# INK-USC/RE-Net

Hardware: NVIDIA H100
Metric: rgcn_aggregate_edge_messages_per_sec (higher is better)
Workload: dtype f32

## Files before the change

renet_b200/csrc/common.cuh:

```cuda
#pragma once
#include <cuda_runtime.h>
#include <stdint.h>
#include <stdio.h>
#include <stdarg.h>

#include "../../include/renet_b200.h"

namespace renet {

void set_error(const char* fmt, ...);
void count_launch(int n = 1);
void note_gemm_kernel(int kernel);
int last_gemm_kernel();

#define RENET_CHECK_ARG(cond, ...)                  \
  do {                                              \
    if (!(cond)) {                                  \
      ::renet::set_error(__VA_ARGS__);              \
      return RENET_ERR_INVALID_ARG;                 \
    }                                               \
  } while (0)

#define RENET_CHECK_CUDA(expr)                                                        \
  do {                                                                                \
    cudaError_t _e = (expr);                                                          \
    if (_e != cudaSuccess) {                                                          \
      ::renet::set_error("%s failed: %s (%s:%d)", #expr, cudaGetErrorString(_e),     \
                         __FILE__, __LINE__);                                         \
      return RENET_ERR_CUDA;                                                          \
    }                                                                                 \
  } while (0)

#define RENET_CHECK_LAUNCH(name)                                                      \
  do {                                                                                \
    cudaError_t _e = cudaGetLastError();                                              \
    if (_e != cudaSuccess) {                                                          \
      ::renet::set_error("launch of %s failed: %s", name, cudaGetErrorString(_e));    \
      return RENET_ERR_CUDA;                                                          \
    }                                                                                 \
    ::renet::count_launch();                                                          \
  } while (0)

constexpr int kNumSMs = 132;

__device__ __forceinline__ float4 ldg_f4(const float* p) {
  return __ldg(reinterpret_cast<const float4*>(p));
}
__device__ __forceinline__ float4 ldg_f4_stream(const float* p) {
  float4 r;
  asm volatile("ld.global.nc.L1::no_allocate.v4.f32 {%0,%1,%2,%3}, [%4];"
               : "=f"(r.x), "=f"(r.y), "=f"(r.z), "=f"(r.w)
               : "l"(p));
  return r;
}
__device__ __forceinline__ void st_f4(float* p, float4 v) { *reinterpret_cast<float4*>(p) = v; }

__device__ __forceinline__ void red_add_f4(float* p, float4 v) {
  asm volatile("red.global.add.v4.f32 [%0], {%1,%2,%3,%4};" ::"l"(p), "f"(v.x), "f"(v.y), "f"(v.z),
               "f"(v.w)
               : "memory");
}

bool deterministic();
int set_deterministic(int on);
int det_scratch(int64_t bytes, cudaStream_t stream, void** out);
int launch_sum_partials(const float* parts, int n_parts, int64_t stride, int64_t rows, int cols, float* out, int64_t ldo,
                        bool accumulate, cudaStream_t stream);
int scatter_add_rows_det(const float* src, int64_t ld, const int32_t* index, const int32_t* outer, float* dst, int64_t n_rows,
                         int d, cudaStream_t stream);

int sgemm_nn(const float* A, const int32_t* a_index, int64_t lda, const float* B, int64_t ldb, float* C,
             int64_t ldc, const float* bias, int64_t M, int32_t N, int32_t K, bool accumulate,
             cudaStream_t stream);
bool sgemm_nn_tiled_ok(const float* A, int64_t lda, const float* B, int64_t ldb, const float* C, int64_t ldc,
                       const float* bias, int32_t N, int32_t K);
int sgemm_nn_ffma(const float* A, const int32_t* a_index, int64_t lda, const float* B, int64_t ldb, float* C,
                  int64_t ldc, const float* bias, int64_t M, int32_t N, int32_t K, bool accumulate, bool naive,
                  cudaStream_t stream);
bool sgemm_tn_tiled_ok(const float* A, int64_t lda, const float* B, int64_t ldb, const float* C, int64_t ldc, int32_t M,
                       int32_t N);
int sgemm_tn(const float* A, const int32_t* a_index, int64_t lda, const float* B, int64_t ldb, float* C,
             int64_t ldc, int32_t M, int32_t N, int64_t K, bool accumulate, cudaStream_t stream, bool naive = false);
int sgemm_nt(const float* A, int64_t lda, const float* B, int64_t ldb, float* C, int64_t ldc,
             int64_t M, int32_t N, int32_t K, bool accumulate, cudaStream_t stream);

int gather_kernel_choice();
constexpr int64_t kStreamMinEdges = 16384;
constexpr int64_t kStreamMinNodes = 16384;
constexpr int64_t kStreamMaxNodes = 40960;
bool gather_use_stream(int64_t E, int64_t N);
void set_stream_debug_buffer(long long* p);

int gemm_mode();
constexpr int64_t kDedupMinRows = 16384;
int64_t umma_packed_bytes(int N, int K);
void set_gemm_debug_buffer(long long* p);
void set_weight_generation(int64_t g);
void* packed_cache_lookup(const void* const* keys, int nkeys, int64_t bytes, bool* hit);
bool umma_shape_ok(int N, int K);
int umma_pack_b(const float* B, int64_t sk, int64_t sn, int N, int K, void* Bp, int tile_offset, cudaStream_t stream);
struct EpiArgs {
  const int32_t* target;
  const float* lse;
  float* pmax;
  float* psum;
  float* tlogit;
  float* dT;
  int64_t ldT;
  float scale;
  const float* dscale;
};
int umma_gemm_prepacked_ex(const float* A, const int32_t* a_index, int64_t lda, const void* Bp, float* C, int64_t ldc,
                           const float* bias, int64_t M, int N, int K, bool accumulate, int batch, int64_t batch_a,
                           int64_t batch_bp, int64_t batch_c, int epi_mode, const EpiArgs& epi, int k_splits, int64_t split_c,
                           cudaStream_t stream);
int umma_gemm_prepacked(const float* A, const int32_t* a_index, int64_t lda, const void* Bp, float* C, int64_t ldc,
                        const float* bias, int64_t M, int N, int K, bool accumulate, int batch, int64_t batch_a,
                        int64_t batch_bp, int64_t batch_c, cudaStream_t stream);
int debug_gemm(int form, int kernel, const float* A, const int32_t* a_index, int64_t lda, const float* B, int64_t ldb, float* C,
               int64_t ldc, const float* bias, int64_t M, int N, int64_t K, bool accumulate, int batch, int64_t batch_a,
               int64_t batch_b, int64_t batch_c, void* ws, int64_t ws_bytes, cudaStream_t stream);

}
```

renet_b200/csrc/rgcn_bwd.cu:

```cuda
#include "common.cuh"
#include "rgcn_tile.cuh"
#include "rgcn_stream.cuh"

namespace renet {
namespace {

constexpr int kWarpsPerCta = 8;

__global__ void relu_mask_kernel(const float* __restrict__ dHout, const float* __restrict__ Hout,
                                 float* __restrict__ P, int64_t n4, int relu) {
  const int64_t i = (int64_t)blockIdx.x * blockDim.x + threadIdx.x;
  if (i >= n4) return;
  float4 g = ldg_f4(dHout + i * 4);
  if (relu) {
    const float4 o = ldg_f4(Hout + i * 4);
    g.x = o.x > 0.f ? g.x : 0.f; g.y = o.y > 0.f ? g.y : 0.f;
    g.z = o.z > 0.f ? g.z : 0.f; g.w = o.w > 0.f ? g.w : 0.f;
  }
  st_f4(P + i * 4, g);
}
__global__ void relu_mask_scalar_kernel(const float* __restrict__ dHout, const float* __restrict__ Hout,
                                        float* __restrict__ P, int64_t n, int relu) {
  const int64_t i = (int64_t)blockIdx.x * blockDim.x + threadIdx.x;
  if (i >= n) return;
  P[i] = (relu && !(Hout[i] > 0.f)) ? 0.f : dHout[i];
}

__global__ void transpose_kernel(const float* __restrict__ src, float* __restrict__ dst, int rows, int cols) {
  __shared__ float tile[32][33];
  const int r0 = blockIdx.x * 32, c0 = blockIdx.y * 32;
  for (int i = threadIdx.y; i < 32; i += 8) {
    int r = r0 + i, c = c0 + threadIdx.x;
    tile[i][threadIdx.x] = (r < rows && c < cols) ? src[(int64_t)r * cols + c] : 0.f;
  }
  __syncthreads();
  for (int i = threadIdx.y; i < 32; i += 8) {
    int c = c0 + i, r = r0 + threadIdx.x;
    if (r < rows && c < cols) dst[(int64_t)c * rows + r] = tile[threadIdx.x][i];
  }
}

template <bool HAS_LOOP, bool DET = false>
__global__ void __launch_bounds__(kTileWarps * 32)
rgcn_dh_tile_kernel(const float* __restrict__ P, const float* __restrict__ W, const int32_t* __restrict__ t_row_ptr,
                    const int32_t* __restrict__ t_col_dst, const int32_t* __restrict__ t_col_type,
                    const float* __restrict__ norm, float* __restrict__ dH, int N) {
  __shared__ __align__(16) float agg[kTileNodes][200];
  __shared__ __align__(16) float head[DET ? kTileWarps : 1][200];
  __shared__ int head_mask[kTileNodes];
  __shared__ int s_rp[kTileNodes + 1];
  const int tid = threadIdx.x;
  const int v0 = blockIdx.x * kTileNodes;
  const int nv = min(kTileNodes, N - v0);
  if (DET) {
    if (tid < kTileNodes) head_mask[tid] = 0;
  } else {
    for (int i = tid; i < kTileNodes * 200; i += kTileWarps * 32) (&agg[0][0])[i] = 0.f;
  }
  if (tid <= nv) s_rp[tid] = __ldg(t_row_ptr + v0 + tid);
  __syncthreads();
  const TileHeads th = DET ? TileHeads{head, head_mask} : TileHeads{nullptr, nullptr};
  tile_accumulate<true, false, true, true, DET>(agg, s_rp, nv, P, nullptr, W, t_col_dst, t_col_type, norm, th);
  __syncthreads();
  for (int i = tid; i < nv * 100; i += kTileWarps * 32) {
    const int r = i / 100, c = (i % 100) * 2;
    float2 o = DET ? tile_row_sum(agg, th, s_rp, r, c) : *reinterpret_cast<const float2*>(&agg[r][c]);
    float* op = dH + (int64_t)(v0 + r) * 200 + c;
    if (HAS_LOOP) {
      const float2 l = *reinterpret_cast<const float2*>(op);
      o.x += l.x; o.y += l.y;
    }
    *reinterpret_cast<float2*>(op) = o;
  }
}

__global__ void rgcn_dh_generic_kernel(const float* __restrict__ P, const float* __restrict__ W,
                                       const int32_t* __restrict__ t_row_ptr, const int32_t* __restrict__ t_col_dst,
                                       const int32_t* __restrict__ t_col_type, const float* __restrict__ norm,
                                       float* __restrict__ dH, int64_t N, int d_in, int d_out, int nb, int has_loop) {
  const int64_t idx = (int64_t)blockIdx.x * blockDim.x + threadIdx.x;
  if (idx >= N * d_in) return;
  const int64_t u = idx / d_in;
  const int c = (int)(idx % d_in);
  const int si = d_in / nb, so = d_out / nb;
  const int b = c / si, i = c % si;
  float acc = 0.f;
  for (int e = t_row_ptr[u]; e < t_row_ptr[u + 1]; ++e) {
    const int64_t d = t_col_dst[e];
    const float* w = W + (int64_t)t_col_type[e] * nb * si * so + (int64_t)b * si * so + (int64_t)i * so;
    const float* g = P + d * d_out + b * so;
    float s = 0.f;
    for (int j = 0; j < so; ++j) s = fmaf(w[j], g[j], s);
    acc = fmaf(s, norm[d], acc);
  }
  dH[idx] = (has_loop ? dH[idx] : 0.f) + acc;
}

constexpr int kEdgesPerWarp = 64;
template <bool INDEXED, bool DET = false>
__global__ void __launch_bounds__(kWarpsPerCta * 32)
rgcn_dw_d200_kernel(const float* __restrict__ H, const int32_t* __restrict__ h_index, const float* __restrict__ P,
                    const int32_t* __restrict__ rel_ptr, const int32_t* __restrict__ rel_src,
                    const int32_t* __restrict__ rel_dst, const float* __restrict__ norm, float* __restrict__ dW,
                    int E, int R2) {
  const int lane = threadIdx.x & 31;
  const int warp = blockIdx.x * kWarpsPerCta + (threadIdx.x >> 5);
  const int e0 = warp * kEdgesPerWarp;
  if (e0 >= E) return;
  const int e1 = min(E, e0 + kEdgesPerWarp);
  const bool active = lane < 25;
  const int foff = lane * 8, woff = lane * 16;
  int lo = 0, hi = R2;
  while (hi - lo > 1) {
    const int mid = (lo + hi) >> 1;
    if (__ldg(rel_ptr + mid) <= e0) lo = mid; else hi = mid;
  }
  int r = lo;
  int r_end = __ldg(rel_ptr + r + 1);
  float acc[16];
#pragma unroll
  for (int i = 0; i < 16; ++i) acc[i] = 0.f;
  float* const wbase = dW + (DET ? (int64_t)warp * 400 : 0) + woff;
  auto flush = [&](int rr) {
    if (active) {
      float* wp = wbase + (int64_t)rr * 400;
#pragma unroll
      for (int k = 0; k < 4; ++k) {
        const float4 v = make_float4(acc[4 * k], acc[4 * k + 1], acc[4 * k + 2], acc[4 * k + 3]);
        if (DET) st_f4(wp + 4 * k, v);
        else red_add_f4(wp + 4 * k, v);
        acc[4 * k] = acc[4 * k + 1] = acc[4 * k + 2] = acc[4 * k + 3] = 0.f;
      }
    }
  };
  for (int base = e0; base < e1; base += 32) {
    const int e = base + lane;
    int my_s = 0, my_d = 0;
    float my_n = 0.f;
    if (e < e1) {
      my_s = __ldg(rel_src + e);
      my_d = __ldg(rel_dst + e);
      my_n = __ldg(norm + my_d);
      if (INDEXED) my_s = __ldg(h_index + my_s);
    }
    const int cnt = min(32, e1 - base);
#pragma unroll 2
    for (int j = 0; j < cnt; ++j) {
      while (base + j >= r_end) {
        flush(r);
        ++r;
        r_end = __ldg(rel_ptr + r + 1);
      }
      const int s = __shfl_sync(0xffffffffu, my_s, j);
      const int d = __shfl_sync(0xffffffffu, my_d, j);
      const float sc = __shfl_sync(0xffffffffu, my_n, j);
      if (active) {
        const float* hp = H + (int64_t)s * 200 + foff;
        const float* gp = P + (int64_t)d * 200 + foff;
        const float4 h0 = ldg_f4_stream(hp), h1 = ldg_f4_stream(hp + 4);
        float4 g0 = ldg_f4_stream(gp), g1 = ldg_f4_stream(gp + 4);
        g0.x *= sc; g0.y *= sc; g0.z *= sc; g0.w *= sc;
        g1.x *= sc; g1.y *= sc; g1.z *= sc; g1.w *= sc;
        acc[0] = fmaf(h0.x, g0.x, acc[0]);  acc[1] = fmaf(h0.x, g0.y, acc[1]);
        acc[2] = fmaf(h0.y, g0.x, acc[2]);  acc[3] = fmaf(h0.y, g0.y, acc[3]);
        acc[4] = fmaf(h0.z, g0.z, acc[4]);  acc[5] = fmaf(h0.z, g0.w, acc[5]);
        acc[6] = fmaf(h0.w, g0.z, acc[6]);  acc[7] = fmaf(h0.w, g0.w, acc[7]);
        acc[8] = fmaf(h1.x, g1.x, acc[8]);  acc[9] = fmaf(h1.x, g1.y, acc[9]);
        acc[10] = fmaf(h1.y, g1.x, acc[10]); acc[11] = fmaf(h1.y, g1.y, acc[11]);
        acc[12] = fmaf(h1.z, g1.z, acc[12]); acc[13] = fmaf(h1.z, g1.w, acc[13]);
        acc[14] = fmaf(h1.w, g1.z, acc[14]); acc[15] = fmaf(h1.w, g1.w, acc[15]);
      }
    }
  }
  flush(r);
}

__global__ void __launch_bounds__(100)
rgcn_dw_reduce_kernel(const float* __restrict__ parts, const int32_t* __restrict__ rel_ptr, float* __restrict__ dW) {
  const int r = blockIdx.x, c = threadIdx.x * 4;
  const int e0 = __ldg(rel_ptr + r), e1 = __ldg(rel_ptr + r + 1);
  if (e0 >= e1) return;
  float* op = dW + (int64_t)r * 400 + c;
  float4 s = *reinterpret_cast<const float4*>(op);
  const int w1 = (e1 - 1) / kEdgesPerWarp;
#pragma unroll 8
  for (int w = e0 / kEdgesPerWarp; w <= w1; ++w) {
    const float4 p = ldg_f4(parts + (int64_t)(w + r) * 400 + c);
    s.x += p.x; s.y += p.y; s.z += p.z; s.w += p.w;
  }
  st_f4(op, s);
}

__global__ void rgcn_dw_generic_kernel(const float* __restrict__ H, const int32_t* __restrict__ h_index,
                                       const float* __restrict__ P, const int32_t* __restrict__ rel_ptr,
                                       const int32_t* __restrict__ rel_src, const int32_t* __restrict__ rel_dst,
                                       const float* __restrict__ norm, float* __restrict__ dW, int R2, int d_in,
                                       int d_out, int nb) {
  const int si = d_in / nb, so = d_out / nb;
  const int per_r = nb * si * so;
  const int64_t idx = (int64_t)blockIdx.x * blockDim.x + threadIdx.x;
  if (idx >= (int64_t)R2 * per_r) return;
  const int r = (int)(idx / per_r), w = (int)(idx % per_r);
  const int b = w / (si * so), i = (w / so) % si, j = w % so;
  float acc = 0.f;
  for (int e = rel_ptr[r]; e < rel_ptr[r + 1]; ++e) {
    int64_t s = rel_src[e];
    if (h_index) s = h_index[s];
    const int64_t d = rel_dst[e];
    acc = fmaf(H[s * d_in + b * si + i], norm[d] * P[d * d_out + b * so + j], acc);
  }
  dW[idx] += acc;
}

__global__ void scatter_add_rows_kernel(const float* __restrict__ src, const int32_t* __restrict__ index,
                                        float* __restrict__ dst, int64_t n_rows, int d4) {
  const int64_t w = ((int64_t)blockIdx.x * blockDim.x + threadIdx.x) >> 5;
  const int lane = threadIdx.x & 31;
  if (w >= n_rows) return;
  const int64_t t = __ldg(index + w);
  for (int i = lane; i < d4; i += 32) red_add_f4(dst + t * d4 * 4 + i * 4, ldg_f4(src + w * d4 * 4 + i * 4));
}
__global__ void scatter_add_rows_scalar_kernel(const float* __restrict__ src, const int32_t* __restrict__ index,
                                               float* __restrict__ dst, int64_t n_rows, int d) {
  const int64_t i = (int64_t)blockIdx.x * blockDim.x + threadIdx.x;
  if (i >= n_rows * d) return;
  atomicAdd(dst + (int64_t)index[i / d] * d + (i % d), src[i]);
}

}

int launch_scatter_add_rows(const float* src, const int32_t* index, float* dst, int64_t n_rows, int d,
                            cudaStream_t stream) {
  if (deterministic()) return scatter_add_rows_det(src, d, index, nullptr, dst, n_rows, d, stream);
  const bool vec = d % 4 == 0 && ((reinterpret_cast<uintptr_t>(src) | reinterpret_cast<uintptr_t>(dst)) & 15) == 0;
  if (vec) {
    const int64_t threads = n_rows * 32;
    scatter_add_rows_kernel<<<(unsigned)((threads + 255) / 256), 256, 0, stream>>>(src, index, dst, n_rows, d / 4);
    RENET_CHECK_LAUNCH("scatter_add_rows_kernel");
  } else {
    const int64_t total = n_rows * d;
    scatter_add_rows_scalar_kernel<<<(unsigned)((total + 255) / 256), 256, 0, stream>>>(src, index, dst, n_rows, d);
    RENET_CHECK_LAUNCH("scatter_add_rows_scalar_kernel");
  }
  return RENET_OK;
}

int launch_selfloop_bwd(const float* H, const int32_t* h_index, const float* Wloop, const float* dLoop, float* dH,
                        float* dWloop, float* WloopT_ws, int64_t N, int d_in, int d_out, cudaStream_t stream) {
  dim3 tg((d_in + 31) / 32, (d_out + 31) / 32);
  transpose_kernel<<<tg, dim3(32, 8), 0, stream>>>(Wloop, WloopT_ws, d_in, d_out);
  RENET_CHECK_LAUNCH("transpose_kernel");
  int rc;
  if ((rc = sgemm_nn(dLoop, nullptr, d_out, WloopT_ws, d_in, dH, d_in, nullptr, N, d_in, d_out, false, stream))) return rc;
  return sgemm_tn(H, h_index, d_in, dLoop, d_out, dWloop, d_out, d_in, d_out, N, true, stream);
}

int launch_rgcn_bwd(const float* H, const int32_t* h_index, const float* W, const float* Wloop,
                    const int32_t* t_row_ptr, const int32_t* t_col_dst, const int32_t* t_col_type,
                    const int32_t* rel_ptr, const int32_t* rel_src, const int32_t* rel_dst, const float* norm,
                    const float* Hout, const float* dHout, float* dH, float* dW, float* dWloop, float* G_ws,
                    int64_t N, int64_t E, int d_in, int d_out, int nb, int R2, int relu, cudaStream_t stream,
                    int64_t N_dst) {
  if (N_dst < 0) N_dst = N;
  float* P = G_ws;
  float* WloopT = G_ws + ((N_dst * d_out + 3) & ~int64_t(3));
  const int64_t n = N_dst * d_out;
  const bool al = ((reinterpret_cast<uintptr_t>(dHout) | reinterpret_cast<uintptr_t>(Hout) |
                    reinterpret_cast<uintptr_t>(P)) & 15) == 0;
  if (n % 4 == 0 && al) {
    relu_mask_kernel<<<(unsigned)((n / 4 + 255) / 256), 256, 0, stream>>>(dHout, Hout, P, n / 4, relu);
    RENET_CHECK_LAUNCH("relu_mask_kernel");
  } else {
    relu_mask_scalar_kernel<<<(unsigned)((n + 255) / 256), 256, 0, stream>>>(dHout, Hout, P, n, relu);
    RENET_CHECK_LAUNCH("relu_mask_scalar_kernel");
  }
  int rc;
  if (Wloop != nullptr) {
    if ((rc = launch_selfloop_bwd(H, h_index, Wloop, P, dH, dWloop, WloopT, N, d_in, d_out, stream))) return rc;
  }
  const bool fast = d_in == 200 && d_out == 200 && nb == 100 &&
                    ((reinterpret_cast<uintptr_t>(H) | reinterpret_cast<uintptr_t>(W) | reinterpret_cast<uintptr_t>(dH) |
                      reinterpret_cast<uintptr_t>(dW) | reinterpret_cast<uintptr_t>(P)) & 15) == 0;
  if (fast) {
    if (E > 0 && gather_use_stream(E, N)) {
      static bool attr_done = false;
      if (!attr_done) {
        RENET_CHECK_CUDA(cudaFuncSetAttribute(rgcn_gather_stream_kernel<false, true, false, true>,
                                              cudaFuncAttributeMaxDynamicSharedMemorySize, StDefault<true>::kSmemBytes));
        RENET_CHECK_CUDA(cudaFuncSetAttribute(rgcn_gather_stream_kernel<false, false, false, true>,
                                              cudaFuncAttributeMaxDynamicSharedMemorySize, StDefault<true>::kSmemBytes));
        attr_done = true;
      }
      if (Wloop != nullptr)
        rgcn_gather_stream_kernel<false, true, false, true><<<kNumSMs, StDefault<true>::kThreads, StDefault<true>::kSmemBytes, stream>>>(
            P, nullptr, W, t_row_ptr, t_col_dst, t_col_type, norm, dH, (int)N, R2, nullptr, 0, (int)E, nullptr);
      else
        rgcn_gather_stream_kernel<false, false, false, true><<<kNumSMs, StDefault<true>::kThreads, StDefault<true>::kSmemBytes, stream>>>(
            P, nullptr, W, t_row_ptr, t_col_dst, t_col_type, norm, dH, (int)N, R2, nullptr, 0, (int)E, nullptr);
      RENET_CHECK_LAUNCH("rgcn_gather_stream_kernel(bwd)");
    } else if (deterministic()) {
      const unsigned grid = (unsigned)((N + kTileNodes - 1) / kTileNodes);
      if (Wloop != nullptr)
        rgcn_dh_tile_kernel<true, true><<<grid, kTileWarps * 32, 0, stream>>>(P, W, t_row_ptr, t_col_dst, t_col_type, norm, dH, (int)N);
      else
        rgcn_dh_tile_kernel<false, true><<<grid, kTileWarps * 32, 0, stream>>>(P, W, t_row_ptr, t_col_dst, t_col_type, norm, dH, (int)N);
      RENET_CHECK_LAUNCH("rgcn_dh_tile_kernel");
    } else {
      const unsigned grid = (unsigned)((N + kTileNodes - 1) / kTileNodes);
      if (Wloop != nullptr)
        rgcn_dh_tile_kernel<true><<<grid, kTileWarps * 32, 0, stream>>>(P, W, t_row_ptr, t_col_dst, t_col_type, norm, dH, (int)N);
      else
        rgcn_dh_tile_kernel<false><<<grid, kTileWarps * 32, 0, stream>>>(P, W, t_row_ptr, t_col_dst, t_col_type, norm, dH, (int)N);
      RENET_CHECK_LAUNCH("rgcn_dh_tile_kernel");
    }
    const int64_t warps = (E + kEdgesPerWarp - 1) / kEdgesPerWarp;
    const unsigned g2 = (unsigned)((warps + kWarpsPerCta - 1) / kWarpsPerCta);
    if (deterministic()) {
      void* parts = nullptr;
      if ((rc = det_scratch((warps + R2) * 400 * (int64_t)sizeof(float), stream, &parts))) return rc;
      float* Wp = static_cast<float*>(parts);
      if (h_index)
        rgcn_dw_d200_kernel<true, true><<<g2, kWarpsPerCta * 32, 0, stream>>>(H, h_index, P, rel_ptr, rel_src, rel_dst, norm, Wp, (int)E, R2);
      else
        rgcn_dw_d200_kernel<false, true><<<g2, kWarpsPerCta * 32, 0, stream>>>(H, h_index, P, rel_ptr, rel_src, rel_dst, norm, Wp, (int)E, R2);
      RENET_CHECK_LAUNCH("rgcn_dw_d200_kernel");
      rgcn_dw_reduce_kernel<<<R2, 100, 0, stream>>>(Wp, rel_ptr, dW);
      RENET_CHECK_LAUNCH("rgcn_dw_reduce_kernel");
      return RENET_OK;
    }
    if (h_index)
      rgcn_dw_d200_kernel<true><<<g2, kWarpsPerCta * 32, 0, stream>>>(H, h_index, P, rel_ptr, rel_src, rel_dst, norm, dW, (int)E, R2);
    else
      rgcn_dw_d200_kernel<false><<<g2, kWarpsPerCta * 32, 0, stream>>>(H, h_index, P, rel_ptr, rel_src, rel_dst, norm, dW, (int)E, R2);
    RENET_CHECK_LAUNCH("rgcn_dw_d200_kernel");
  } else {
    const int64_t t1 = N * d_in;
    rgcn_dh_generic_kernel<<<(unsigned)((t1 + 255) / 256), 256, 0, stream>>>(P, W, t_row_ptr, t_col_dst, t_col_type,
                                                                            norm, dH, N, d_in, d_out, nb, Wloop != nullptr);
    RENET_CHECK_LAUNCH("rgcn_dh_generic_kernel");
    const int64_t t2 = (int64_t)R2 * nb * (d_in / nb) * (d_out / nb);
    rgcn_dw_generic_kernel<<<(unsigned)((t2 + 255) / 256), 256, 0, stream>>>(H, h_index, P, rel_ptr, rel_src, rel_dst,
                                                                            norm, dW, R2, d_in, d_out, nb);
    RENET_CHECK_LAUNCH("rgcn_dw_generic_kernel");
  }
  return RENET_OK;
}

}
```

renet_b200/csrc/rgcn_fwd.cu:

```cuda
#include <stdlib.h>

#include "common.cuh"
#include "rgcn_tile.cuh"
#include "rgcn_stream.cuh"

namespace renet {
namespace {

template <bool RELU, bool HAS_LOOP, bool INDEXED, int NODES = kTileNodes>
__global__ void __launch_bounds__(kTileWarps * 32, 768 / (kTileWarps * 32))
rgcn_gather_d200_kernel(const float* __restrict__ H, const int32_t* __restrict__ h_index,
                        const float* __restrict__ W, const int32_t* __restrict__ row_ptr,
                        const int32_t* __restrict__ col_src, const int32_t* __restrict__ col_type,
                        const float* __restrict__ norm, float* __restrict__ Hout, int N, int passthrough) {
  __shared__ __align__(16) float agg[NODES][200];
  __shared__ __align__(16) float loopbuf[HAS_LOOP ? NODES : 1][200];
  __shared__ __align__(16) float head[kTileWarps][200];
  __shared__ int head_mask[NODES];
  __shared__ float normbuf[NODES];
  __shared__ int s_rp[NODES + 1];
  const int tid = threadIdx.x;
  const int v0 = blockIdx.x * NODES;
  const int nv = min(NODES, N - v0);
  tile_prefetch_epilogue(loopbuf, normbuf, Hout + (int64_t)v0 * 200, norm + v0, nv, HAS_LOOP, tid, kTileWarps * 32);
  if (tid < NODES) head_mask[tid] = 0;
  if (tid <= nv) s_rp[tid] = __ldg(row_ptr + v0 + tid);
  __syncthreads();
  const TileHeads th{head, head_mask};
  tile_accumulate<false, INDEXED, false, true, true>(agg, s_rp, nv, H, h_index, W, col_src, col_type, nullptr, th);
  cp_async_wait_all();
  __syncthreads();
  for (int i = tid; i < nv * 100; i += kTileWarps * 32) {
    const int r = i / 100, c = (i % 100) * 2;
    const int v = v0 + r;
    float2 a = tile_row_sum(agg, th, s_rp, r, c);
    if (passthrough) {
      const int64_t hr = INDEXED ? (int64_t)__ldg(h_index + v) : v;
      a = *reinterpret_cast<const float2*>(H + hr * 200 + c);
    }
    const float nvv = normbuf[r];
    float* op = Hout + (int64_t)v * 200 + c;
    float2 o = make_float2(a.x * nvv, a.y * nvv);
    if (HAS_LOOP) {
      const float2 l = *reinterpret_cast<const float2*>(&loopbuf[r][c]);
      o.x += l.x; o.y += l.y;
    }
    if (RELU) { o.x = fmaxf(o.x, 0.f); o.y = fmaxf(o.y, 0.f); }
    *reinterpret_cast<float2*>(op) = o;
  }
}

__global__ void rgcn_gather_generic_kernel(const float* __restrict__ H, const int32_t* __restrict__ h_index,
                                           const float* __restrict__ W, const int32_t* __restrict__ row_ptr,
                                           const int32_t* __restrict__ col_src,
                                           const int32_t* __restrict__ col_type, const float* __restrict__ norm,
                                           float* __restrict__ Hout, int64_t N, int d_in, int d_out, int nb,
                                           int relu, int has_loop, int passthrough) {
  const int64_t i = (int64_t)blockIdx.x * blockDim.x + threadIdx.x;
  if (i >= N * d_out) return;
  const int64_t v = i / d_out;
  const int c = (int)(i % d_out);
  const int si = d_in / nb, so = d_out / nb;
  const int b = c / so, j = c % so;
  float acc = 0.f;
  for (int e = row_ptr[v]; e < row_ptr[v + 1]; ++e) {
    int64_t s = col_src[e];
    if (h_index) s = h_index[s];
    const float* w = W + (int64_t)col_type[e] * nb * si * so + (int64_t)b * si * so + j;
    const float* h = H + s * d_in + b * si;
    for (int k = 0; k < si; ++k) acc = fmaf(h[k], w[k * so], acc);
  }
  if (passthrough) {
    const int64_t r = h_index ? (int64_t)h_index[v] : v;
    acc = H[r * d_in + c];
  }
  float o = acc * norm[v];
  if (has_loop) o += Hout[i];
  if (relu) o = fmaxf(o, 0.f);
  Hout[i] = o;
}

}

int gather_kernel_choice() {
  static int v = -1;
  if (v < 0) {
    const char* e = getenv("RENET_GATHER_KERNEL");
    v = 0;
    if (e && e[0] == 't') v = 1;
    else if (e && e[0] == 's') v = 3;
  }
  return v;
}
bool gather_use_stream(int64_t E, int64_t N) {
  const int c = gather_kernel_choice();
  return c == 3 || (c == 0 && E >= kStreamMinEdges && N >= kStreamMinNodes && N <= kStreamMaxNodes);
}

static long long* g_stream_dbg = nullptr;
void set_stream_debug_buffer(long long* p) { g_stream_dbg = p; }

int stream_cfg_choice() {
  static int v = -1;
  if (v < 0) {
    const char* e = getenv("RENET_STREAM_CFG");
    v = e ? atoi(e) : 0;
  }
  return v;
}

template <bool RELU, bool HAS_LOOP, bool INDEXED, class Cfg>
static int launch_stream_cfg(const float* H, const int32_t* h_index, const float* W, const int32_t* row_ptr,
                             const int32_t* col_src, const int32_t* col_type, const float* norm, float* Hout, int N, int R2,
                             const int32_t* hot_rel, int n_hot, int E_hint, cudaStream_t stream) {
  static bool attr_done = false;
  if (!attr_done) {
    RENET_CHECK_CUDA(cudaFuncSetAttribute(rgcn_gather_stream_kernel<RELU, HAS_LOOP, INDEXED, false, Cfg>,
                                          cudaFuncAttributeMaxDynamicSharedMemorySize, Cfg::kSmemBytes));
    attr_done = true;
  }
  long long* dbg = g_stream_dbg;
  rgcn_gather_stream_kernel<RELU, HAS_LOOP, INDEXED, false, Cfg><<<kNumSMs, Cfg::kThreads, Cfg::kSmemBytes, stream>>>(
      H, h_index, W, row_ptr, col_src, col_type, norm, Hout, N, R2, hot_rel, n_hot, E_hint, dbg);
  RENET_CHECK_LAUNCH("rgcn_gather_stream_kernel");
  return RENET_OK;
}

template <bool RELU, bool HAS_LOOP, bool INDEXED>
static int launch_stream(const float* H, const int32_t* h_index, const float* W, const int32_t* row_ptr,
                         const int32_t* col_src, const int32_t* col_type, const float* norm, float* Hout, int N, int R2,
                         const int32_t* hot_rel, int n_hot, int E_hint, cudaStream_t stream) {
#define RENET_ST(...) return launch_stream_cfg<RELU, HAS_LOOP, INDEXED, __VA_ARGS__>(H, h_index, W, row_ptr, col_src, col_type, norm, Hout, N, R2, hot_rel, n_hot, E_hint, stream)
  if (RELU && HAS_LOOP) {
    switch (stream_cfg_choice()) {
      case 1: RENET_ST(StCfg<28, 2, 31, false>);
      case 2: RENET_ST(StCfg<24, 2, 44, false>);
      default: break;
    }
  }
  RENET_ST(StDefault<false>);
#undef RENET_ST
}

int launch_rgcn_gather(const float* H, const int32_t* h_index, const float* W, const int32_t* row_ptr,
                       const int32_t* col_src, const int32_t* col_type, const float* norm, float* Hout,
                       int64_t N, int64_t E, int d_in, int d_out, int nb, int relu, int has_loop,
                       cudaStream_t stream, int R2, const int32_t* hot_rel, int n_hot) {
  if (N == 0) return RENET_OK;
  const int passthrough = (E == 0) ? 1 : 0;
  const bool fast = d_in == 200 && d_out == 200 && nb == 100 &&
                    ((reinterpret_cast<uintptr_t>(H) | reinterpret_cast<uintptr_t>(W) |
                      reinterpret_cast<uintptr_t>(Hout)) & 15) == 0;
  if (fast) {
    const int key = (relu ? 4 : 0) | (has_loop ? 2 : 0) | (h_index ? 1 : 0);
    if (!passthrough && gather_use_stream(E, N)) {
#define RENET_LAUNCH_STREAM(R, L, I) return launch_stream<R, L, I>(H, h_index, W, row_ptr, col_src, col_type, norm, Hout, (int)N, R2, hot_rel, n_hot, (int)E, stream)
      switch (key) {
        case 0: RENET_LAUNCH_STREAM(false, false, false);
        case 1: RENET_LAUNCH_STREAM(false, false, true);
        case 2: RENET_LAUNCH_STREAM(false, true, false);
        case 3: RENET_LAUNCH_STREAM(false, true, true);
        case 4: RENET_LAUNCH_STREAM(true, false, false);
        case 5: RENET_LAUNCH_STREAM(true, false, true);
        case 6: RENET_LAUNCH_STREAM(true, true, false);
        default: RENET_LAUNCH_STREAM(true, true, true);
      }
#undef RENET_LAUNCH_STREAM
    }
    const unsigned block = kTileWarps * 32;
    const unsigned n_tiles = (unsigned)((N + kTileNodes - 1) / kTileNodes);
#define RENET_LAUNCH_GATHER(R, L, I)                                                                            \
    rgcn_gather_d200_kernel<R, L, I><<<n_tiles, block, 0, stream>>>(H, h_index, W, row_ptr, col_src, col_type, norm, Hout, (int)N, passthrough)
    switch (key) {
      case 0: RENET_LAUNCH_GATHER(false, false, false); break;
      case 1: RENET_LAUNCH_GATHER(false, false, true); break;
      case 2: RENET_LAUNCH_GATHER(false, true, false); break;
      case 3: RENET_LAUNCH_GATHER(false, true, true); break;
      case 4: RENET_LAUNCH_GATHER(true, false, false); break;
      case 5: RENET_LAUNCH_GATHER(true, false, true); break;
      case 6: RENET_LAUNCH_GATHER(true, true, false); break;
      default: RENET_LAUNCH_GATHER(true, true, true); break;
    }
#undef RENET_LAUNCH_GATHER
    RENET_CHECK_LAUNCH("rgcn_gather_d200_kernel");
  } else {
    const int64_t total = N * d_out;
    rgcn_gather_generic_kernel<<<(unsigned)((total + 255) / 256), 256, 0, stream>>>(
        H, h_index, W, row_ptr, col_src, col_type, norm, Hout, N, d_in, d_out, nb, relu, has_loop, passthrough);
    RENET_CHECK_LAUNCH("rgcn_gather_generic_kernel");
  }
  return RENET_OK;
}

}
```

renet_b200/csrc/rgcn_stream.cuh:

```cuda
#pragma once
#include <type_traits>

#include "common.cuh"
#include "umma.cuh"

namespace renet {

constexpr int kStRpCap = 1024;
constexpr int kStMaxR2 = 2048;
constexpr int kStNodeCost = 2;
constexpr int kStSlot = 800;
constexpr int kStHotGroups = 8;
template <int WARPS, int D, int HOT, bool BWD>
struct StCfg {
  static constexpr int kWarps = WARPS, kThreads = WARPS * 32, kD = D, kHot = HOT;
  static constexpr int kHotPerGroup = (HOT + kStHotGroups - 1) / kStHotGroups;
  static constexpr int kBlk = (32 / D) * D;
  static constexpr int kOffRing = 0;
  static constexpr int kOffHot = kOffRing + WARPS * D * kStSlot;
  static constexpr int kOffHeads = kOffHot + HOT * 1600;
  static constexpr int kOffRp = kOffHeads + WARPS * 800;
  static constexpr int kOffSlotOf = kOffRp + kStRpCap * 4;
  static constexpr int kOffIdx = kOffSlotOf + kStMaxR2;
  static constexpr int kOffSc = kOffIdx + WARPS * 64 * 8;
  static constexpr int kOffBars = kOffSc + (BWD ? WARPS * 64 * 4 : 0);
  static constexpr int kOffFlags = kOffBars + (WARPS * D + kStHotGroups + WARPS) * 8;
  static constexpr int kSmemBytes = kOffFlags + (2 * WARPS + 17) * 4;
  static_assert(WARPS >= 16 && WARPS <= 32, "stream gather: the partition search needs 512 threads");
  static_assert(kBlk == 32, "stream gather: index blocks are 32 edges (D = 2 or 4)");
  static_assert(kSmemBytes <= 227 * 1024, "stream gather: shared memory budget");
  static_assert(WARPS * D * kStSlot >= (kStMaxR2 + 256 + 8) * 4, "stream gather: prologue scratch lives in the ring");
  static_assert(HOT <= 254 && (kOffHot + HOT * 1600) / 16 < 65536, "stream gather: hot rows are addressed by 16-bit offsets");
};
template <bool BWD>
using StDefault = StCfg<32, 2, BWD ? 77 : 82, BWD>;

namespace {

__device__ __forceinline__ void st_bulk_g2s(uint32_t dst, const void* src, uint32_t bytes, uint32_t bar) {
  asm volatile("cp.async.bulk.shared::cluster.global.mbarrier::complete_tx::bytes [%0], [%1], %2, [%3];" ::"r"(dst), "l"(src),
               "r"(bytes), "r"(bar)
               : "memory");
}
__device__ __forceinline__ void st_expect_tx(uint32_t bar, uint32_t bytes) {
  asm volatile("mbarrier.arrive.expect_tx.shared::cta.b64 _, [%0], %1;" ::"r"(bar), "r"(bytes) : "memory");
}
__device__ __forceinline__ bool st_elect_one() {
  uint32_t pred;
  asm volatile(
      "{\n"
      ".reg .pred p;\n"
      "elect.sync _|p, 0xffffffff;\n"
      "selp.u32 %0, 1, 0, p;\n"
      "}\n"
      : "=r"(pred));
  return pred != 0;
}
__device__ __forceinline__ void st_wait(uint32_t bar, uint32_t parity) {
  uint32_t done;
  asm volatile(
      "{\n"
      ".reg .pred p;\n"
      "mbarrier.try_wait.parity.shared::cta.b64 p, [%1], %2;\n"
      "selp.u32 %0, 1, 0, p;\n"
      "}\n"
      : "=r"(done)
      : "r"(bar), "r"(parity)
      : "memory");
  if (!done) mbar_wait(bar, parity);
}
template <int OFF>
__device__ __forceinline__ float2 st_lds_f2(uint32_t a) {
  float2 r;
  asm volatile("ld.shared.v2.f32 {%0,%1}, [%2+%3];" : "=f"(r.x), "=f"(r.y) : "r"(a), "n"(OFF));
  return r;
}
template <int OFF>
__device__ __forceinline__ float4 st_lds_f4(uint32_t a) {
  float4 r;
  asm volatile("ld.shared.v4.f32 {%0,%1,%2,%3}, [%4+%5];" : "=f"(r.x), "=f"(r.y), "=f"(r.z), "=f"(r.w) : "r"(a), "n"(OFF));
  return r;
}
__device__ __forceinline__ uint32_t st_lds_u32(uint32_t a) {
  uint32_t r;
  asm volatile("ld.shared.u32 %0, [%1];" : "=r"(r) : "r"(a));
  return r;
}
__device__ __forceinline__ uint32_t st_opaque(uint32_t v) {
  asm volatile("" : "+r"(v));
  return v;
}
__device__ __forceinline__ void st_arrive(uint32_t bar) {
  asm volatile("mbarrier.arrive.shared::cta.b64 _, [%0];" ::"r"(bar) : "memory");
}

}

template <bool RELU, bool HAS_LOOP, bool INDEXED, bool BWD, class Cfg = StDefault<BWD>>
__global__ void __launch_bounds__(Cfg::kThreads, 1)
rgcn_gather_stream_kernel(const float* __restrict__ X, const int32_t* __restrict__ x_index, const float* __restrict__ W,
                          const int32_t* __restrict__ row_ptr, const int32_t* __restrict__ col_a,
                          const int32_t* __restrict__ col_type, const float* __restrict__ norm, float* __restrict__ Hout,
                          int N, int R2, const int32_t* __restrict__ hot_rel, int n_hot_arg, int E_hint,
                          long long* __restrict__ dbg) {
  extern __shared__ __align__(128) uint8_t st_smem[];
  auto stamp = [&](int k, long long v) {
    if (dbg && (threadIdx.x & 31) == 0) dbg[((int64_t)blockIdx.x * Cfg::kWarps + (threadIdx.x >> 5)) * 8 + k] = v;
  };
  auto global_timer = []() {
    long long t;
    asm volatile("mov.u64 %0, %%globaltimer;" : "=l"(t));
    return t;
  };
  if (dbg) { stamp(0, clock64()); stamp(5, global_timer()); }
  constexpr int D = Cfg::kD, kBlk = Cfg::kBlk, kStWarps = Cfg::kWarps, kStThreads = Cfg::kThreads;
  float* heads = reinterpret_cast<float*>(st_smem + Cfg::kOffHeads);
  int32_t* s_rp = reinterpret_cast<int32_t*>(st_smem + Cfg::kOffRp);
  uint8_t* slot_of = st_smem + Cfg::kOffSlotOf;
  int* flags = reinterpret_cast<int*>(st_smem + Cfg::kOffFlags);
  int* s_part = flags + kStWarps;
  int* s_e0 = s_part + 16;
  uint64_t* bars = reinterpret_cast<uint64_t*>(st_smem + Cfg::kOffBars);
  int* cnt = reinterpret_cast<int*>(st_smem + Cfg::kOffRing);
  int* hist = cnt + kStMaxR2;

  const int tid = threadIdx.x, lane = tid & 31;
  const int warp = __shfl_sync(0xffffffffu, tid >> 5, 0);
  const bool tail4 = lane < 4;
  const bool use_hot = R2 > 0 && R2 <= kStMaxR2 && Cfg::kHot > 0;
  const bool given_hot = use_hot && hot_rel != nullptr;
  {
    const int64_t gt = (int64_t)blockIdx.x * Cfg::kThreads + threadIdx.x;
    const int64_t n_rp_lines = ((int64_t)N + 1 + 31) / 32, n_e_lines = ((int64_t)E_hint + 31) / 32;
    const char* pf = nullptr;
    if (gt < n_rp_lines) pf = reinterpret_cast<const char*>(row_ptr) + gt * 128;
    else if (gt < n_rp_lines + n_e_lines) pf = reinterpret_cast<const char*>(col_a) + (gt - n_rp_lines) * 128;
    else if (gt < n_rp_lines + 2 * n_e_lines) pf = reinterpret_cast<const char*>(col_type) + (gt - n_rp_lines - n_e_lines) * 128;
    else if (INDEXED && gt < 2 * n_rp_lines + 2 * n_e_lines - 1)
      pf = reinterpret_cast<const char*>(x_index) + (gt - n_rp_lines - 2 * n_e_lines) * 128;
    if (pf) asm volatile("prefetch.global.L2 [%0];" ::"l"(pf));
  }
  const int E = __ldg(row_ptr + N);
  const uint32_t hot_bar0 = smem_u32(bars + kStWarps * D);
  const uint32_t head_bar0 = hot_bar0 + kStHotGroups * 8;

  if (tid < 16) s_part[tid] = 0;
  if (tid < kStWarps) flags[tid] = 0;
  if (lane == 0) {
#pragma unroll
    for (int k = 0; k < D; ++k) mbar_init(smem_u32(bars + warp * D + k), 1);
    mbar_init(head_bar0 + warp * 8, 1);
    if (warp == 0)
      for (int gr = 0; gr < kStHotGroups; ++gr) mbar_init(hot_bar0 + gr * 8, 1);
    asm volatile("fence.mbarrier_init.release.cluster;" ::: "memory");
  }
  if (!given_hot)
    for (int i = tid; i < kStMaxR2 + 256; i += kStThreads) cnt[i] = 0;
  for (int i = tid; i < kStMaxR2 / 4; i += kStThreads) reinterpret_cast<uint32_t*>(slot_of)[i] = 0u;
  __syncthreads();
  auto load_hot = [&](int n_hot, auto row_of) {
    if (lane < kStHotGroups) {
      const int rows = min(max(n_hot - lane * Cfg::kHotPerGroup, 0), Cfg::kHotPerGroup);
      st_expect_tx(hot_bar0 + lane * 8, (uint32_t)rows * 1600u);
    }
    __syncwarp();
    for (int sl = lane; sl < n_hot; sl += 32)
      st_bulk_g2s(smem_u32(st_smem + Cfg::kOffHot + sl * 1600), W + (int64_t)row_of(sl) * 400, 1600,
                  hot_bar0 + (sl / Cfg::kHotPerGroup) * 8);
  };
  if (given_hot && warp == 1) {
    load_hot(min(n_hot_arg, Cfg::kHot), [&](int sl) {
      const int r = __ldg(hot_rel + sl);
      const bool ok = r >= 0 && r < R2;
      if (ok) slot_of[r] = (uint8_t)(sl + 1);
      return ok ? r : 0;
    });
  }
  const int half = tid >> 8, ht = tid & 255;
  const int c_idx = blockIdx.x + half;
  const int64_t total_cost = (int64_t)E + (int64_t)kStNodeCost * N;
  const int64_t target = ((int64_t)c_idx * total_cost) / gridDim.x;
  const bool searching = tid < 512 && c_idx > 0 && c_idx < (int)gridDim.x;
  int lo = 0, hi = N;
  const int rounds = N < 256 ? 1 : (N < 65536 ? 2 : (N < (1 << 24) ? 3 : 4));
  for (int r = 0; r < rounds; ++r) {
    const int step = (hi - lo) / 256 + 1;
    const int p = min(lo + (ht + 1) * step - 1, hi);
    const int val = searching ? __ldg(row_ptr + p) : 0;
    const bool below = searching && (int64_t)val + (int64_t)kStNodeCost * p < target;
    const unsigned m = __ballot_sync(0xffffffffu, below);
    if (lane == 0 && m) atomicAdd(&s_part[2 * r + (half & 1)], __popc(m));
    __syncthreads();
    const int f = s_part[2 * r + (half & 1)];
    if (r == rounds - 1 && searching) {
      if (ht == f) { s_part[10 + half] = lo + f; s_part[12 + half] = val; }
      if (ht == f - 1) s_part[14 + half] = val + 1;
    }
    const int new_hi = min(lo + (f + 1) * step - 1, hi);
    const int new_lo = f == 0 ? lo : min(lo + f * step - 1, hi) + 1;
    lo = new_lo; hi = new_hi;
  }
  __syncthreads();
  int A = 0, A_next = N, cb = 0, ce = E;
  if (blockIdx.x > 0) {
    A = s_part[10]; cb = s_part[12];
    const int64_t tgt = ((int64_t)blockIdx.x * total_cost) / gridDim.x;
    const int64_t k_hi = (int64_t)cb + (int64_t)kStNodeCost * A, k_lo = (int64_t)(s_part[14] - 1) + (int64_t)kStNodeCost * (A - 1);
    if (s_part[14] && k_hi - tgt > tgt - k_lo) { --A; cb = s_part[14] - 1; }
  }
  if (blockIdx.x + 1 < gridDim.x) {
    A_next = s_part[11]; ce = s_part[13];
    const int64_t tgt = ((int64_t)(blockIdx.x + 1) * total_cost) / gridDim.x;
    const int64_t k_hi = (int64_t)ce + (int64_t)kStNodeCost * A_next, k_lo = (int64_t)(s_part[15] - 1) + (int64_t)kStNodeCost * (A_next - 1);
    if (s_part[15] && k_hi - tgt > tgt - k_lo) { --A_next; ce = s_part[15] - 1; }
  }
  if (dbg) stamp(1, clock64());
  const int n_rp = A_next - A + 1;
  const bool rp_in_smem = n_rp <= kStRpCap;
  auto rp = [&](int v) -> int { return rp_in_smem ? s_rp[v - A] : __ldg(row_ptr + v); };
  if (rp_in_smem)
    for (int i = tid; i < n_rp; i += kStThreads) s_rp[i] = __ldg(row_ptr + A + i);
  __syncthreads();
  const int64_t cta_cost = (int64_t)(ce - cb) + (int64_t)kStNodeCost * (A_next - A);
  auto range_start = [&](int j) -> int {
    const int64_t T = (cta_cost * j) / kStWarps;
    int l = A, h = A_next;
    while (l < h) {
      const int mid = (l + h + 1) >> 1;
      if ((int64_t)(rp(mid) - cb) + (int64_t)kStNodeCost * (mid - A) <= T) l = mid; else h = mid - 1;
    }
    if (l >= A_next) return ce;
    const int64_t r = T - ((int64_t)(rp(l) - cb) + (int64_t)kStNodeCost * (l - A));
    return rp(l) + (int)min(r, (int64_t)(rp(l + 1) - rp(l)));
  };
  const int e0 = range_start(warp), e1 = warp + 1 < kStWarps ? range_start(warp + 1) : ce;
  const int n = e1 - e0;
  if (lane == 0) { s_e0[warp] = e0; if (warp == kStWarps - 1) s_e0[kStWarps] = ce; }

  int2* my_idx = reinterpret_cast<int2*>(st_smem + Cfg::kOffIdx) + warp * 64;
  float* my_sc = reinterpret_cast<float*>(st_smem + Cfg::kOffSc) + warp * 64;
  int ld_s = 0, ld_t = 0;
  float ld_sc = 1.f;
  auto block_load = [&](int b) {
    const int e = e0 + b * kBlk + lane;
    ld_s = 0; ld_t = 0; ld_sc = 1.f;
    if (lane < kBlk && e < e1) {
      ld_s = __ldg(col_a + e);
      ld_t = __ldg(col_type + e);
    }
  };
  auto block_gather = [&](int b) {
    const int e = e0 + b * kBlk + lane;
    if ((BWD || INDEXED) && lane < kBlk && e < e1) {
      if (BWD) ld_sc = __ldg(norm + ld_s);
      if (INDEXED) ld_s = __ldg(x_index + ld_s);
    }
  };
  auto block_stage = [&](int b) {
    const int hs = use_hot ? (int)slot_of[ld_t] : 0;
    const int woff16 = hs ? (Cfg::kOffHot + (hs - 1) * 1600) >> 4 : 0;
    my_idx[(b & 1) * 32 + lane] = make_int2(ld_s, hs ? (woff16 << 16) | ((hs - 1) / Cfg::kHotPerGroup) : ld_t);
    if (BWD) my_sc[(b & 1) * 32 + lane] = ld_sc;
    __syncwarp();
  };
  block_load(0);

  if (use_hot && !given_hot) {
    for (int e = e0 + lane; e < e1; e += 32) atomicAdd(&cnt[__ldg(col_type + e)], 1);
    __syncthreads();
    for (int r = tid; r < R2; r += kStThreads) {
      const int c = cnt[r];
      if (c > 0) atomicAdd(&hist[min(c, 255)], 1);
    }
    __syncthreads();
    if (warp == 0) {
      int s = 0;
#pragma unroll
      for (int k = 0; k < 8; ++k) s += hist[lane * 8 + k];
      int suf = s;
#pragma unroll
      for (int d = 1; d < 32; d <<= 1) {
        const int o = __shfl_down_sync(0xffffffffu, suf, d);
        if (lane + d < 32) suf += o;
      }
      int running = suf - s, thr = 256;
#pragma unroll
      for (int k = 7; k >= 0; --k) {
        running += hist[lane * 8 + k];
        if (running <= Cfg::kHot && lane * 8 + k >= 1) thr = lane * 8 + k;
      }
#pragma unroll
      for (int d = 16; d >= 1; d >>= 1) thr = min(thr, __shfl_xor_sync(0xffffffffu, thr, d));
      if (lane == 0) s_part[8] = thr;
    }
    __syncthreads();
    const int thr = s_part[8];
    for (int r = tid; r < R2; r += kStThreads) {
      if (min(cnt[r], 255) >= thr) {
        const int slot = atomicAdd(&s_part[9], 1);
        slot_of[r] = (uint8_t)(slot + 1);
        hist[slot] = r;
      }
    }
    __syncthreads();
    if (thr > 1) {
      for (int r = tid; r < R2; r += kStThreads) {
        if (min(cnt[r], 255) == thr - 1) {
          const int slot = atomicAdd(&s_part[9], 1);
          if (slot < Cfg::kHot) { slot_of[r] = (uint8_t)(slot + 1); hist[slot] = r; }
        }
      }
      __syncthreads();
    }
    if (warp == 1) load_hot(min(s_part[9], Cfg::kHot), [&](int sl) { return hist[sl]; });
  }
  block_gather(0);
  __syncthreads();
  block_stage(0);
  block_load(1);

  const uint32_t ring = st_opaque(smem_u32(st_smem + Cfg::kOffRing + warp * D * kStSlot));
  const uint32_t bar0 = st_opaque(smem_u32(bars + warp * D));
  const uint32_t idx_a = st_opaque(smem_u32(my_idx));
  auto issue = [&](int k, int slot) {
    if (st_elect_one()) {
      const uint32_t src = st_lds_u32(idx_a + (((uint32_t)k & 63u) << 3));
      const uint32_t bar = bar0 + slot * 8;
      st_expect_tx(bar, 800u);
      st_bulk_g2s(ring + slot * kStSlot, X + (int64_t)(int)src * 200, 800, bar);
    }
  };
  asm volatile("griddepcontrol.wait;" ::: "memory");
#pragma unroll
  for (int k = 0; k < D; ++k)
    if (k < n) issue(k, k);

  int va;
  {
    int l = A, h = A_next;
    while (h > l) {
      const int mid = (l + h) >> 1;
      if (rp(mid) >= e0) h = mid; else l = mid + 1;
    }
    va = l;
  }
  int cur = va;
  bool continued = false;
  if (n > 0 && rp(va) > e0) { cur = va - 1; continued = true; }
  int cur_end = cur < A_next ? rp(cur + 1) : ce;
  float acc[8];
#pragma unroll
  for (int i = 0; i < 8; ++i) acc[i] = 0.f;
  float2 lp[4];
  float nrm = 1.f;
#pragma unroll
  for (int k = 0; k < 4; ++k) lp[k] = make_float2(0.f, 0.f);
  auto fetch_dest = [&](int v) {
    if (v < A_next) {
      if (HAS_LOOP) {
#pragma unroll
        for (int k = 0; k < 4; ++k)
          if (k < 3 || tail4) lp[k] = *reinterpret_cast<const float2*>(Hout + (int64_t)v * 200 + 2 * (lane + 32 * k));
      }
      if (!BWD) nrm = __ldg(norm + v);
    }
  };
  auto epilogue = [&](int v) {
#pragma unroll
    for (int k = 0; k < 4; ++k) {
      if (k < 3 || tail4) {
        float2 o = make_float2(acc[2 * k], acc[2 * k + 1]);
        if (!BWD) { o.x *= nrm; o.y *= nrm; }
        if (HAS_LOOP) { o.x += lp[k].x; o.y += lp[k].y; }
        if (RELU) { o.x = fmaxf(o.x, 0.f); o.y = fmaxf(o.y, 0.f); }
        *reinterpret_cast<float2*>(Hout + (int64_t)v * 200 + 2 * (lane + 32 * k)) = o;
      }
    }
#pragma unroll
    for (int i = 0; i < 8; ++i) acc[i] = 0.f;
  };
  auto publish_head = [&]() {
#pragma unroll
    for (int k = 0; k < 4; ++k)
      if (k < 3 || tail4)
        *reinterpret_cast<float2*>(heads + warp * 200 + 2 * (lane + 32 * k)) = make_float2(acc[2 * k], acc[2 * k + 1]);
    __syncwarp();
    if (lane == 0) st_arrive(head_bar0 + warp * 8);
#pragma unroll
    for (int i = 0; i < 8; ++i) acc[i] = 0.f;
  };
  int cur_beg = cur < A_next ? rp(cur) : ce;
  auto advance = [&]() {
    if (continued) { publish_head(); continued = false; }
    else if (cur_end > cur_beg) epilogue(cur);
    ++cur;
    cur_beg = cur_end;
    cur_end = cur < A_next ? rp(cur + 1) : ce;
    fetch_dest(cur);
  };
  if (!continued) fetch_dest(cur);

  const uint32_t ring_l8 = st_opaque(ring + 8 * lane);
  const uint32_t smem_l16 = st_opaque(smem_u32(st_smem) + 16 * lane);
  const float* w_l4 = W + 4 * lane;
  uint32_t hot_seen = 0;
  const uint32_t sc_a = BWD ? st_opaque(smem_u32(my_sc)) : 0u;
  uint32_t parity = 0;
  constexpr int kP1 = (kBlk / D / 3) * D, kP2 = (2 * (kBlk / D) / 3) * D;
  int phase_at = kP1, phase = 0, blk = 0;
  if (dbg) stamp(2, clock64());
  for (int g = 0; g < n; g += D) {
    if (g == phase_at) {
      if (phase == 0) { block_gather(blk + 1); phase_at += kP2 - kP1; phase = 1; }
      else if (phase == 1) { block_stage(blk + 1); phase_at += kBlk - kP2; phase = 2; }
      else { ++blk; block_load(blk + 1); phase_at += kP1; phase = 0; }
    }
    auto do_slot = [&](auto slot_c) {
      constexpr int slot = decltype(slot_c)::value;
      const int i = g + slot;
      if (i < n) {
        while (e0 + i >= cur_end) advance();
        const uint32_t wsel = st_lds_u32(idx_a + (((uint32_t)i & 63u) << 3) + 4);
        const uint32_t woff16 = wsel >> 16;
        const float sc = BWD ? __uint_as_float(st_lds_u32(sc_a + (((uint32_t)i & 63u) << 2))) : 1.f;
        float2 h[4];
        float4 w[4];
        w[3] = make_float4(0.f, 0.f, 0.f, 0.f);
        if (woff16) {
          const uint32_t grp = wsel & 0xffffu;
          if (!((hot_seen >> grp) & 1u)) { mbar_wait(hot_bar0 + grp * 8, 0); hot_seen |= 1u << grp; }
          const uint32_t wa = smem_l16 + (woff16 << 4);
          w[0] = st_lds_f4<0>(wa); w[1] = st_lds_f4<512>(wa); w[2] = st_lds_f4<1024>(wa);
          if (tail4) w[3] = st_lds_f4<1536>(wa);
        } else {
          const float* wr = w_l4 + (int64_t)(int)wsel * 400;
          w[0] = ldg_f4(wr); w[1] = ldg_f4(wr + 128); w[2] = ldg_f4(wr + 256);
          if (tail4) w[3] = ldg_f4(wr + 384);
        }
        st_wait(bar0 + slot * 8, parity);
        h[0] = st_lds_f2<slot * kStSlot>(ring_l8);       h[1] = st_lds_f2<slot * kStSlot + 256>(ring_l8);
        h[2] = st_lds_f2<slot * kStSlot + 512>(ring_l8);
        h[3] = make_float2(0.f, 0.f);
        if (tail4) h[3] = st_lds_f2<slot * kStSlot + 768>(ring_l8);
#pragma unroll
        for (int k = 0; k < 4; ++k) {
          const float x = BWD ? h[k].x * sc : h[k].x, y = BWD ? h[k].y * sc : h[k].y;
          if (!BWD) {
            acc[2 * k] = fmaf(x, w[k].x, fmaf(y, w[k].z, acc[2 * k]));
            acc[2 * k + 1] = fmaf(x, w[k].y, fmaf(y, w[k].w, acc[2 * k + 1]));
          } else {
            acc[2 * k] = fmaf(x, w[k].x, fmaf(y, w[k].y, acc[2 * k]));
            acc[2 * k + 1] = fmaf(x, w[k].z, fmaf(y, w[k].w, acc[2 * k + 1]));
          }
        }
        __syncwarp();
        if (i + D < n) issue(i + D, slot);
      }
    };
    do_slot(std::integral_constant<int, 0>{});
    do_slot(std::integral_constant<int, 1>{});
    if constexpr (D == 4) {
      do_slot(std::integral_constant<int, 2>{});
      do_slot(std::integral_constant<int, 3>{});
    }
    parity ^= 1u;
  }
  if (dbg) stamp(3, clock64());
  if (n > 0) {
    if (cur_end <= e1) {
      advance();
    } else if (continued) {
      publish_head();
      ++cur;
    } else {
      for (int k = warp + 1; k < kStWarps && s_e0[k] < cur_end; ++k) {
        if (s_e0[k + 1] == s_e0[k]) continue;
        mbar_wait(head_bar0 + k * 8, 0);
#pragma unroll
        for (int q = 0; q < 4; ++q) {
          if (q < 3 || tail4) {
            const float2 hv = *reinterpret_cast<const float2*>(heads + k * 200 + 2 * (lane + 32 * q));
            acc[2 * q] += hv.x; acc[2 * q + 1] += hv.y;
          }
        }
      }
      epilogue(cur);
      ++cur;
    }
  }
  for (int base = (blockIdx.x * kStWarps + warp) * 32; base < N; base += gridDim.x * kStWarps * 32) {
    const int v = base + lane;
    const bool iso = v < N && __ldg(row_ptr + v) == __ldg(row_ptr + v + 1);
    unsigned m = __ballot_sync(0xffffffffu, iso);
    while (m) {
      const int u = base + __ffs(m) - 1;
      m &= m - 1;
#pragma unroll
      for (int k = 0; k < 4; ++k) {
        if (k < 3 || tail4) {
          float* op = Hout + (int64_t)u * 200 + 2 * (lane + 32 * k);
          float2 o = make_float2(0.f, 0.f);
          if (HAS_LOOP) o = *reinterpret_cast<const float2*>(op);
          if (RELU) { o.x = fmaxf(o.x, 0.f); o.y = fmaxf(o.y, 0.f); }
          if (RELU || !HAS_LOOP) *reinterpret_cast<float2*>(op) = o;
        }
      }
    }
  }
  if (dbg) { stamp(4, clock64()); stamp(6, global_timer()); stamp(7, n); }
}

}
```

Measured before the change: 2.532 billion.

## Lower stream-kernel node threshold for plain inputs and overlap hot-relation loads with partition search

Result: faster. 2.622 billion, median of 6 (+3.5%).

```diff
diff --git a/renet_b200/csrc/common.cuh b/renet_b200/csrc/common.cuh
--- a/renet_b200/csrc/common.cuh
+++ b/renet_b200/csrc/common.cuh
@@ -87,8 +87,9 @@
 int gather_kernel_choice();
 constexpr int64_t kStreamMinEdges = 16384;
 constexpr int64_t kStreamMinNodes = 16384;
+constexpr int64_t kStreamMinPlainNodes = 2048;
 constexpr int64_t kStreamMaxNodes = 40960;
-bool gather_use_stream(int64_t E, int64_t N);
+bool gather_use_stream(int64_t E, int64_t N, bool indexed_input);
 void set_stream_debug_buffer(long long* p);
 
 int gemm_mode();
diff --git a/renet_b200/csrc/rgcn_bwd.cu b/renet_b200/csrc/rgcn_bwd.cu
--- a/renet_b200/csrc/rgcn_bwd.cu
+++ b/renet_b200/csrc/rgcn_bwd.cu
@@ -282,7 +282,7 @@
                     ((reinterpret_cast<uintptr_t>(H) | reinterpret_cast<uintptr_t>(W) | reinterpret_cast<uintptr_t>(dH) |
                       reinterpret_cast<uintptr_t>(dW) | reinterpret_cast<uintptr_t>(P)) & 15) == 0;
   if (fast) {
-    if (E > 0 && gather_use_stream(E, N)) {
+    if (E > 0 && gather_use_stream(E, N, true)) {
       static bool attr_done = false;
       if (!attr_done) {
         RENET_CHECK_CUDA(cudaFuncSetAttribute(rgcn_gather_stream_kernel<false, true, false, true>,
diff --git a/renet_b200/csrc/rgcn_fwd.cu b/renet_b200/csrc/rgcn_fwd.cu
--- a/renet_b200/csrc/rgcn_fwd.cu
+++ b/renet_b200/csrc/rgcn_fwd.cu
@@ -92,9 +92,10 @@
   }
   return v;
 }
-bool gather_use_stream(int64_t E, int64_t N) {
+bool gather_use_stream(int64_t E, int64_t N, bool indexed_input) {
   const int c = gather_kernel_choice();
-  return c == 3 || (c == 0 && E >= kStreamMinEdges && N >= kStreamMinNodes && N <= kStreamMaxNodes);
+  const int64_t min_nodes = indexed_input ? kStreamMinNodes : kStreamMinPlainNodes;
+  return c == 3 || (c == 0 && E >= kStreamMinEdges && N >= min_nodes && N <= kStreamMaxNodes);
 }
 
 static long long* g_stream_dbg = nullptr;
@@ -153,7 +154,7 @@
                       reinterpret_cast<uintptr_t>(Hout)) & 15) == 0;
   if (fast) {
     const int key = (relu ? 4 : 0) | (has_loop ? 2 : 0) | (h_index ? 1 : 0);
-    if (!passthrough && gather_use_stream(E, N)) {
+    if (!passthrough && gather_use_stream(E, N, h_index != nullptr)) {
 #define RENET_LAUNCH_STREAM(R, L, I) return launch_stream<R, L, I>(H, h_index, W, row_ptr, col_src, col_type, norm, Hout, (int)N, R2, hot_rel, n_hot, (int)E, stream)
       switch (key) {
         case 0: RENET_LAUNCH_STREAM(false, false, false);
diff --git a/renet_b200/csrc/rgcn_stream.cuh b/renet_b200/csrc/rgcn_stream.cuh
--- a/renet_b200/csrc/rgcn_stream.cuh
+++ b/renet_b200/csrc/rgcn_stream.cuh
@@ -42,6 +42,9 @@
                "r"(bytes), "r"(bar)
                : "memory");
 }
+__device__ __forceinline__ void st_cp_async4(uint32_t dst, const void* src) {
+  asm volatile("cp.async.ca.shared.global [%0], [%1], 4;" ::"r"(dst), "l"(src) : "memory");
+}
 __device__ __forceinline__ void st_expect_tx(uint32_t bar, uint32_t bytes) {
   asm volatile("mbarrier.arrive.expect_tx.shared::cta.b64 _, [%0], %1;" ::"r"(bar), "r"(bytes) : "memory");
 }
@@ -141,6 +144,17 @@
     if (pf) asm volatile("prefetch.global.L2 [%0];" ::"l"(pf));
   }
   const int E = __ldg(row_ptr + N);
+  const int half = tid >> 8, ht = tid & 255;
+  const int c_idx = blockIdx.x + half;
+  const bool searching = tid < 512 && c_idx > 0 && c_idx < (int)gridDim.x;
+  const int probe0 = min((ht + 1) * (N / 256 + 1) - 1, N);
+  const int val0 = searching ? __ldg(row_ptr + probe0) : 0;
+  constexpr int kHotIters = (Cfg::kHot + 31) / 32;
+  const int n_hot_given = given_hot ? min(n_hot_arg, Cfg::kHot) : 0;
+  if (warp == 1) {
+    for (int sl = lane; sl < n_hot_given; sl += 32) st_cp_async4(smem_u32(hist + sl), hot_rel + sl);
+    asm volatile("cp.async.commit_group;" ::: "memory");
+  }
   const uint32_t hot_bar0 = smem_u32(bars + kStWarps * D);
   const uint32_t head_bar0 = hot_bar0 + kStHotGroups * 8;
 
@@ -164,29 +178,22 @@
       st_expect_tx(hot_bar0 + lane * 8, (uint32_t)rows * 1600u);
     }
     __syncwarp();
-    for (int sl = lane; sl < n_hot; sl += 32)
-      st_bulk_g2s(smem_u32(st_smem + Cfg::kOffHot + sl * 1600), W + (int64_t)row_of(sl) * 400, 1600,
-                  hot_bar0 + (sl / Cfg::kHotPerGroup) * 8);
-  };
-  if (given_hot && warp == 1) {
-    load_hot(min(n_hot_arg, Cfg::kHot), [&](int sl) {
-      const int r = __ldg(hot_rel + sl);
-      const bool ok = r >= 0 && r < R2;
-      if (ok) slot_of[r] = (uint8_t)(sl + 1);
-      return ok ? r : 0;
-    });
-  }
-  const int half = tid >> 8, ht = tid & 255;
-  const int c_idx = blockIdx.x + half;
+#pragma unroll
+    for (int k = 0; k < kHotIters; ++k) {
+      const int sl = lane + 32 * k;
+      if (sl < n_hot)
+        st_bulk_g2s(smem_u32(st_smem + Cfg::kOffHot + sl * 1600), W + (int64_t)row_of(k) * 400, 1600,
+                    hot_bar0 + (sl / Cfg::kHotPerGroup) * 8);
+    }
+  };
   const int64_t total_cost = (int64_t)E + (int64_t)kStNodeCost * N;
   const int64_t target = ((int64_t)c_idx * total_cost) / gridDim.x;
-  const bool searching = tid < 512 && c_idx > 0 && c_idx < (int)gridDim.x;
   int lo = 0, hi = N;
   const int rounds = N < 256 ? 1 : (N < 65536 ? 2 : (N < (1 << 24) ? 3 : 4));
   for (int r = 0; r < rounds; ++r) {
     const int step = (hi - lo) / 256 + 1;
     const int p = min(lo + (ht + 1) * step - 1, hi);
-    const int val = searching ? __ldg(row_ptr + p) : 0;
+    const int val = r == 0 ? val0 : (searching ? __ldg(row_ptr + p) : 0);
     const bool below = searching && (int64_t)val + (int64_t)kStNodeCost * p < target;
     const unsigned m = __ballot_sync(0xffffffffu, below);
     if (lane == 0 && m) atomicAdd(&s_part[2 * r + (half & 1)], __popc(m));
@@ -201,6 +208,15 @@
     lo = new_lo; hi = new_hi;
   }
   __syncthreads();
+  if (given_hot && warp == 1) {
+    asm volatile("cp.async.wait_all;" ::: "memory");
+    load_hot(n_hot_given, [&](int k) {
+      const int sl = lane + 32 * k, r = hist[sl];
+      const bool ok = r >= 0 && r < R2;
+      if (ok) slot_of[r] = (uint8_t)(sl + 1);
+      return ok ? r : 0;
+    });
+  }
   int A = 0, A_next = N, cb = 0, ce = E;
   if (blockIdx.x > 0) {
     A = s_part[10]; cb = s_part[12];
@@ -312,7 +328,7 @@
       }
       __syncthreads();
     }
-    if (warp == 1) load_hot(min(s_part[9], Cfg::kHot), [&](int sl) { return hist[sl]; });
+    if (warp == 1) load_hot(min(s_part[9], Cfg::kHot), [&](int k) { return hist[lane + 32 * k]; });
   }
   block_gather(0);
   __syncthreads();
```
